# JuliaReinforcementLearning/ReinforcementLearning.jl

Measured on NVIDIA H100. Metric: env-steps/sec at 65536 CartPole envs (full PPO iteration: rollout T=32 + GAE + 4 epochs x 4 minibatches), higher is better.
Workload: dtype f32

## Files before the change

### reinforcementlearning.jl_b200/csrc/nn_tc.cu

```cuda
#include "nn.cuh"
#include "perm.cuh"
#include "policy.cuh"
#include "tc_fwd.cuh"
#include "tc_split.h"
#include "wgmma.cuh"

namespace {

using tcfwd::G_F;
using tcfwd::GW_S;
using tcfwd::WIMG_BYTES;
using tcfwd::split2;
using tcfwd::wimg_off;
constexpr int TM = tcfwd::TM;
constexpr int H = tcfwd::H;
constexpr float kScaleW = tcfwd::kScale;

constexpr int NT7 = 512;
constexpr int kMaxStage = 10;
constexpr int GF_T = 128;
constexpr int GS_T = 16 * GF_T;
constexpr int FIMG = 8 * GS_T;
constexpr float kScaleH = 64.0f, kScaleX = 64.0f;
constexpr int kNo = 2;

struct SmemBwd {
    static_assert(FIMG % 128 == 0 && WIMG_BYTES % 128 == 0 && (2 * GS_T) % 16 == 0, "operand images must stay 128-byte aligned");
    alignas(128) uint8_t FP_full[FIMG];
    alignas(128) uint8_t FP_lo[FIMG];
    alignas(128) uint8_t AH[2][2][FIMG];
    alignas(128) uint8_t FQ_full[FIMG];
    alignas(128) uint8_t FQ_lo[FIMG];
    alignas(128) uint8_t B1[WIMG_BYTES];
    alignas(128) uint8_t XT[2][2 * GS_T];
    alignas(16) float D[TM * H];
    uint64_t H1pos[2][TM];
    float W1[kInMax * H];
    float b1[H], b2[H];
    float W3[H * kNo];
    float b3[kNo];
    float Zp[4 * kNo * TM];
    float Red[32];
    double RedD[16];
    float step_scale;
    alignas(8) uint64_t bar1[2];
    alignas(8) uint64_t bar3;
    alignas(8) uint64_t bar4;
    float AccW2[64 * 65 + 64];
    float AccD4[64 * 9];
};
__device__ __forceinline__ int d_off(int s, int col) { return s * H + ((((col >> 2) ^ (s & 15))) << 2) + (col & 3); }
__device__ __forceinline__ void d_ld16(const float* D, int s, int f0, float (&v)[16]) {
#pragma unroll
    for (int u = 0; u < 4; ++u) {
        const float4 q4 = *reinterpret_cast<const float4*>(D + d_off(s, f0 + 4 * u));
        v[4 * u] = q4.x; v[4 * u + 1] = q4.y; v[4 * u + 2] = q4.z; v[4 * u + 3] = q4.w;
    }
}
template <int TB>
__device__ __forceinline__ void gemm_ts3(float (&d)[32], const uint8_t* a_hi, const uint8_t* a_lo, int h, uint64_t dB, uint32_t b_step) {
    const uint64_t dA = wg::make_desc(wg::smem_u32(a_hi) + 8 * h * GF_T, GS_T, GF_T), dAl = wg::make_desc(wg::smem_u32(a_lo) + 8 * h * GF_T, GS_T, GF_T);
    wg::fence();
#pragma unroll
    for (int k = 0; k < 4; ++k) {
        const uint32_t aa = k * 2 * GS_T, bb = k * b_step;
        wg::mma_m64n64k16<0, TB>(d, wg::desc_add(dA, aa), wg::desc_add(dB, bb), k ? 1u : 0u);
        wg::mma_m64n64k16<0, TB>(d, wg::desc_add(dA, aa), wg::desc_add(dB, 8 * GW_S + bb), 1u);
        wg::mma_m64n64k16<0, TB>(d, wg::desc_add(dAl, aa), wg::desc_add(dB, bb), 1u);
    }
    wg::commit();
    wg::wait_all();
}
__device__ __forceinline__ uint32_t fimg_off(int f, int s) { return (uint32_t)((f >> 3) * GS_T + (s >> 3) * GF_T + (s & 7) * 16 + (f & 7) * 2); }
__device__ __forceinline__ void store16_feat(uint8_t* img, int f0, int s, const uint32_t (&v)[8]) {
    uint8_t* p = img + fimg_off(f0, s);
    *reinterpret_cast<uint4*>(p) = make_uint4(v[0], v[1], v[2], v[3]);
    *reinterpret_cast<uint4*>(p + GS_T) = make_uint4(v[4], v[5], v[6], v[7]);
}
using b200perm::perm_index;
using b200perm::perm_index_bits;

__device__ __forceinline__ float lane_transpose_reduce32(float (&v)[32], int lane) {
#pragma unroll
    for (int st = 0; st < 5; ++st) {
        const int half = 16 >> st, off = 16 >> st;
        const bool upper = (lane & off) != 0;
#pragma unroll
        for (int n = 0; n < half; ++n) {
            float send = upper ? v[n] : v[n + half];
            float keep = upper ? v[n + half] : v[n];
            v[n] = keep + __shfl_xor_sync(0xffffffffu, send, off);
        }
    }
    return v[0];
}

__device__ __forceinline__ void worker_sync() { asm volatile("bar.sync 1, 512;" ::: "memory"); }
__device__ __forceinline__ void group_sync(int q) { asm volatile("bar.sync %0, 128;" ::"r"(5 + q) : "memory"); }
__device__ __forceinline__ void ready_arrive(int id) { asm volatile("bar.arrive %0, 384;" ::"r"(id) : "memory"); }
__device__ __forceinline__ void ready_wait(int id) { asm volatile("bar.sync %0, 384;" ::"r"(id) : "memory"); }
#ifdef B200RL_K7_TIMING
__device__ unsigned long long g_k7_phase[40];
__device__ int g_k7_watch = 0;
#define K7_T(i) do { if (tid == (g_k7_watch & 0xFFFF) && (int)blockIdx.x == (g_k7_watch >> 16)) { long long now_ = clock64(); g_k7_phase[i] += (unsigned long long)(now_ - tprev_); tprev_ = now_; } } while (0)
#else
#define K7_T(i) do { } while (0)
#endif
constexpr int NT7_ALL = NT7 + 128;
constexpr int kRegsMma = 64, kRegsWorker = 104;
static_assert(128 * kRegsMma + NT7 * kRegsWorker <= NT7_ALL * 96, "setmaxnreg split must fit the CTA's register allocation");
constexpr int kBarRdyA = 2, kBarRdyB = 9;
constexpr int kBarMma = 4;
__device__ __forceinline__ void mma_sync() { asm volatile("bar.sync %0, 128;" ::"n"(kBarMma) : "memory"); }

template <int ACT>
__global__ void __launch_bounds__(NT7_ALL, 1)
ac_loss_grad_tc_kernel(MlpDesc actor, MlpDesc critic, const float* params , AcHyper hp, AcBatch b, float* partial,
                       float* __restrict__ loss_partial, int64_t np_total, float scale_base ,
                       OptStep st ,
                       int n_actor ) {
    extern __shared__ __align__(1024) unsigned char smem_raw[];
    SmemBwd& sm = *reinterpret_cast<SmemBwd*>(smem_raw);
    const int role = (int)blockIdx.x < n_actor ? 0 : 1;
    const int cta = role ? (int)blockIdx.x - n_actor : (int)blockIdx.x;
    const int nctas = role ? (int)gridDim.x - n_actor : n_actor;
    const int nrows = max(n_actor, (int)gridDim.x - n_actor);
    const float scale_p = scale_base * (role ? 4.0f : 64.0f);
    const MlpDesc d = role ? critic : actor;
    const int act = ACT >= 0 ? ACT : d.act;
    const bool relu = act == B200RL_ACT_RELU;
    const int64_t poff = role ? actor.nparams() : 0;
    const float* __restrict__ p = params + poff;
    const int tid = threadIdx.x, warp = tid >> 5, lane = tid & 31;
    const int q = warp & 3, c = (warp >> 2) & 3;
    const int s = 32 * q + lane;
    const int half = q >> 1;
    {
        const float* b1 = p + (int64_t)H * d.in;
        const float* W2 = b1 + H;
        const float* b2 = W2 + (int64_t)H * H;
        const float s1 = relu ? kScaleH : 1.0f;
        for (int k = tid; k < kInMax * H; k += NT7_ALL) sm.W1[k] = (k / H) < d.in ? p[k] * s1 : 0.f;
        for (int k = tid; k < H; k += NT7_ALL) { sm.b1[k] = b1[k] * s1; sm.b2[k] = b2[k]; }
        for (int k = tid; k < H * kNo; k += NT7_ALL) {
            int j = k / kNo, o = k % kNo;
            sm.W3[k] = o < d.nout ? p[head_w<false>(d, o, j)] : 0.f;
        }
        if (tid < kNo) sm.b3[tid] = tid < d.nout ? p[head_b<false>(d, tid)] : 0.f;
        tcfwd::fill_w2_image<NT7_ALL>(sm.B1, W2);
    }
    if (tid == 32) {
        wg::mbar_init(&sm.bar1[0], 128); wg::mbar_init(&sm.bar1[1], 128); wg::mbar_init(&sm.bar3, 128); wg::mbar_init(&sm.bar4, 128);
    }
    wg::fence_proxy_async();
    __syncthreads();
    const float inv_s1 = 1.0f / (kScaleH * kScaleW), inv_s3 = 1.0f / (scale_p * kScaleH), inv_sp = 1.0f / scale_p, inv_s4 = 1.0f / (scale_p * kScaleX);
    const int64_t ntiles = (b.B + TM - 1) / TM;

    if (warp >= NT7 / 32) {
        asm volatile("setmaxnreg.dec.sync.aligned.u32 %0;" ::"n"(kRegsMma));
        const int t = tid - NT7, row0 = 16 * (t >> 5) + ((t & 31) >> 2), col0 = 2 * (t & 3);
        const uint64_t dB1k = wg::make_desc(wg::smem_u32(sm.B1), G_F, GW_S);
        const uint64_t dB1t = wg::make_desc(wg::smem_u32(sm.B1), GW_S, G_F);
        float dacc[32];
        auto store_d = [&](int h) {
#pragma unroll
            for (int j = 0; j < 8; ++j)
#pragma unroll
                for (int hh = 0; hh < 2; ++hh)
                    *reinterpret_cast<float2*>(sm.D + d_off(64 * h + row0 + 8 * hh, 8 * j + col0)) = make_float2(dacc[4 * j + 2 * hh], dacc[4 * j + 2 * hh + 1]);
        };
        auto gemm1 = [&](int h, int buf) { gemm_ts3<0>(dacc, sm.AH[buf][0], sm.AH[buf][1], h, dB1k, 2 * G_F); };
        auto gemm2 = [&](int h) { gemm_ts3<1>(dacc, sm.FP_full, sm.FP_lo, h, dB1t, 2 * GW_S); };
        auto store_dp1 = [&](int h, int pbuf) {
#pragma unroll
            for (int hh = 0; hh < 2; ++hh) {
                const int ss = 64 * h + row0 + 8 * hh;
                const uint64_t pos = relu ? sm.H1pos[pbuf][ss] >> col0 : 0u;
#pragma unroll
                for (int j = 0; j < 8; ++j) {
                    const uint32_t off = fimg_off(8 * j + col0, ss);
                    float v0 = dacc[4 * j + 2 * hh] * (1.0f / kScaleW), v1 = dacc[4 * j + 2 * hh + 1] * (1.0f / kScaleW);
                    if (relu) {
                        v0 = ((pos >> (8 * j)) & 1u) ? v0 : 0.f;
                        v1 = ((pos >> (8 * j + 1)) & 1u) ? v1 : 0.f;
                    } else {
                        const float inv_h = 1.0f / kScaleH;
                        const float2 hf = __half22float2(*reinterpret_cast<const __half2*>(sm.AH[pbuf][0] + off));
                        const float2 lf = __half22float2(*reinterpret_cast<const __half2*>(sm.AH[pbuf][1] + off));
                        v0 *= dact_f(act, (hf.x + lf.x) * inv_h);
                        v1 *= dact_f(act, (hf.y + lf.y) * inv_h);
                    }
                    uint32_t hi, lo;
                    split2(v0, v1, hi, lo);
                    *reinterpret_cast<uint32_t*>(sm.FQ_full + off) = hi;
                    *reinterpret_cast<uint32_t*>(sm.FQ_lo + off) = lo;
                }
            }
        };
        auto gemm3 = [&](int buf) {
            const uint64_t dPh = wg::make_desc(wg::smem_u32(sm.FP_full), GF_T, GS_T), dPl = wg::make_desc(wg::smem_u32(sm.FP_lo), GF_T, GS_T);
            const uint64_t dHh = wg::make_desc(wg::smem_u32(sm.AH[buf][0]), GF_T, GS_T), dHl = wg::make_desc(wg::smem_u32(sm.AH[buf][1]), GF_T, GS_T);
            wg::fence();
#pragma unroll
            for (int k = 0; k < 8; ++k) {
                const uint32_t a = k * 2 * GF_T;
                wg::mma_m64n64k16<1, 1>(dacc, wg::desc_add(dPh, a), wg::desc_add(dHh, a), k ? 1u : 0u);
                wg::mma_m64n64k16<1, 1>(dacc, wg::desc_add(dPl, a), wg::desc_add(dHh, a), 1u);
                wg::mma_m64n64k16<1, 1>(dacc, wg::desc_add(dPh, a), wg::desc_add(dHl, a), 1u);
            }
            wg::commit();
            wg::wait_all();
#pragma unroll
            for (int j = 0; j < 8; ++j)
#pragma unroll
                for (int hh = 0; hh < 2; ++hh)
#pragma unroll
                    for (int e = 0; e < 2; ++e) sm.AccW2[(row0 + 8 * hh) * 65 + 8 * j + col0 + e] += dacc[4 * j + 2 * hh + e];
            const uint64_t dX = wg::make_desc(wg::smem_u32(sm.XT[buf]), GF_T, GS_T);
            float d8[4] = {0.f, 0.f, 0.f, 0.f};
            wg::fence();
#pragma unroll
            for (int k = 0; k < 8; ++k) {
                const uint32_t a = k * 2 * GF_T;
                wg::mma_m64n8k16<1, 1>(d8, wg::desc_add(dPh, a), wg::desc_add(dX, a), k ? 1u : 0u);
                wg::mma_m64n8k16<1, 1>(d8, wg::desc_add(dPl, a), wg::desc_add(dX, a), 1u);
            }
            wg::commit();
            wg::wait_all();
            if (col0 == 4) {
                sm.AccW2[64 * 65 + row0] += d8[0];
                sm.AccW2[64 * 65 + row0 + 8] += d8[2];
            }
        };
        auto gemm4 = [&](int buf) {
            const uint64_t dQh = wg::make_desc(wg::smem_u32(sm.FQ_full), GF_T, GS_T), dQl = wg::make_desc(wg::smem_u32(sm.FQ_lo), GF_T, GS_T);
            const uint64_t dX = wg::make_desc(wg::smem_u32(sm.XT[buf]), GF_T, GS_T);
            float d4[4] = {0.f, 0.f, 0.f, 0.f};
            wg::fence();
#pragma unroll
            for (int k = 0; k < 8; ++k) {
                const uint32_t a = k * 2 * GF_T;
                wg::mma_m64n8k16<1, 1>(d4, wg::desc_add(dQh, a), wg::desc_add(dX, a), k ? 1u : 0u);
                wg::mma_m64n8k16<1, 1>(d4, wg::desc_add(dQh, a), wg::desc_add(dX, GS_T + a), 1u);
                wg::mma_m64n8k16<1, 1>(d4, wg::desc_add(dQl, a), wg::desc_add(dX, a), 1u);
            }
            wg::commit();
            wg::wait_all();
#pragma unroll
            for (int hh = 0; hh < 2; ++hh)
#pragma unroll
                for (int e = 0; e < 2; ++e)
                    if (col0 + e < 5) sm.AccD4[(row0 + 8 * hh) * 9 + col0 + e] += d4[2 * hh + e];
        };
        if (cta < ntiles) {
            for (int h = 0; h < 2; ++h) {
                ready_wait(kBarRdyB + h);
                gemm1(h, 0); store_d(h);
                wg::mbar_arrive(&sm.bar1[h]);
            }
        }
        int buf = 0;
        for (int64_t tile = cta; tile < ntiles; tile += nctas, buf ^= 1) {
            const bool has_next = tile + nctas < ntiles;
            for (int h = 0; h < 2; ++h) {
                ready_wait(kBarRdyA + h);
                gemm2(h); store_dp1(h, buf);
                if (has_next) {
                    ready_wait(kBarRdyB + h);
                    gemm1(h, buf ^ 1); store_d(h);
                    wg::mbar_arrive(&sm.bar1[h]);
                }
            }
            wg::fence_proxy_async();
            gemm3(buf);
            wg::mbar_arrive(&sm.bar3);
            mma_sync();
            gemm4(buf);
            wg::mbar_arrive(&sm.bar4);
        }
    } else {
    asm volatile("setmaxnreg.inc.sync.aligned.u32 %0;" ::"n"(kRegsWorker));
    float g3[2][16];
    float gb3a0 = 0.f, gb3a1 = 0.f;
#pragma unroll
    for (int k = 0; k < 16; ++k) { g3[0][k] = 0.f; g3[1][k] = 0.f; }
    float l0 = 0.f, l1 = 0.f;
    float mean = 0.f, inv_std = 1.f;
    if (hp.normalize_adv && b.norm2) { mean = b.norm2[0]; inv_std = b.norm2[1]; }
    uint32_t ph1 = 0, ph3 = 0, ph4 = 0;
    bool gemm4_pending = false;
    int xbuf = 0;
    int pbuf = 0;
#ifdef B200RL_K7_TIMING
    long long tprev_ = clock64();
#endif
    const int pbits = b200perm::perm_bits(b.perm_n);
    const uint32_t pkey = ac_perm_key(b);
    auto index_of = [&](int64_t t) -> int32_t {
        const int64_t j = t * TM + s;
        if (t >= ntiles || j >= b.B) return -1;
        return b.idx ? b.idx[j] : (int32_t)perm_index_bits((uint32_t)(b.perm_offset + j), b.perm_n, pkey, pbits);
    };
    auto request = [&](int32_t g, float (&x)[kInMax], float (&a)[4]) {
#pragma unroll
        for (int k = 0; k < kInMax; ++k) { x[k] = 0.f; a[k] = 0.f; }
        if (g < 0) return;
        if (b.rec) {
            const float4 v0 = b.rec[2 * (int64_t)g], v1 = b.rec[2 * (int64_t)g + 1];
            x[0] = v0.x; x[1] = v0.y; x[2] = v0.z; x[3] = v0.w;
            a[0] = v1.x; a[1] = v1.y; a[2] = v1.z; a[3] = v1.w;
        } else {
#pragma unroll
            for (int i = 0; i < kInMax; ++i)
                if (i < b.ns) x[i] = b.states[(int64_t)b.ns * g + i];
            a[0] = reinterpret_cast<const float*>(b.actions)[g];
            a[1] = b.logp_old ? b.logp_old[g] : 0.f;
            a[2] = b.adv[g];
            a[3] = b.ret[g];
        }
    };
    float pfx[kInMax] = {0.f, 0.f, 0.f, 0.f}, pfa[4] = {0.f, 0.f, 0.f, 0.f};
    float aux[4] = {0.f, 0.f, 0.f, 0.f};
    int32_t gi_next = -1;
    bool gemm3_pending = false;
    float* const out = partial + (int64_t)cta * np_total + poff;
    float* const gW1 = out;
    float* const gb1 = out + (int64_t)H * d.in;
    float* const gW2 = gb1 + H;
    float* const gb2 = gW2 + (int64_t)H * H;
    for (int k = tid; k < 64 * 65 + 64; k += NT7) sm.AccW2[k] = 0.f;
    for (int k = tid; k < 64 * 9; k += NT7) sm.AccD4[k] = 0.f;
    float xo[kInMax];
    auto publish = [&](int64_t t) {
#pragma unroll
        for (int i = 0; i < kInMax; ++i) xo[i] = pfx[i];
        aux[0] = pfa[0];
        aux[1] = role == 0 ? pfa[1] : 0.f;
        aux[2] = role == 0 ? (hp.normalize_adv ? (pfa[2] - mean) * inv_std : pfa[2]) : 0.f;
        aux[3] = role == 0 ? 0.f : pfa[3];
        if (c == 0) {
            uint32_t h01, l01, h23, l23;
            split2(xo[0] * kScaleX, xo[1] * kScaleX, h01, l01);
            split2(xo[2] * kScaleX, xo[3] * kScaleX, h23, l23);
            uint8_t* xt = sm.XT[xbuf] + fimg_off(0, s);
            *reinterpret_cast<uint4*>(xt) = make_uint4(h01, h23, 0x3C00u, 0u);
            *reinterpret_cast<uint4*>(xt + GS_T) = make_uint4(l01, l23, 0u, 0u);
        }
        K7_T(16);
        xbuf ^= 1;
        request(gi_next, pfx, pfa);
        gi_next = index_of(t + 2 * nctas);
        K7_T(17);
    };
    auto layer1 = [&]() {
        uint32_t pos = 0;
        uint32_t hi8[8], lo8[8];
#pragma unroll
        for (int ch = 0; ch < 4; ++ch) {
            const int f0 = 16 * c + 4 * ch;
            float4 bb = *reinterpret_cast<const float4*>(sm.b1 + f0);
            float h[4] = {bb.x, bb.y, bb.z, bb.w};
#pragma unroll
            for (int k = 0; k < kInMax; ++k) {
                float4 w = *reinterpret_cast<const float4*>(sm.W1 + k * H + f0);
                h[0] = fmaf(w.x, xo[k], h[0]); h[1] = fmaf(w.y, xo[k], h[1]); h[2] = fmaf(w.z, xo[k], h[2]); h[3] = fmaf(w.w, xo[k], h[3]);
            }
            if (relu) {
#pragma unroll
                for (int e = 0; e < 4; ++e) { pos |= (h[e] > 0.f ? 1u : 0u) << (4 * ch + e); h[e] = fmaxf(h[e], 0.f); }
            } else {
#pragma unroll
                for (int e = 0; e < 4; ++e) h[e] = act_f(act, h[e]) * kScaleH;
            }
            split2(h[0], h[1], hi8[2 * ch], lo8[2 * ch]);
            split2(h[2], h[3], hi8[2 * ch + 1], lo8[2 * ch + 1]);
        }
        if (relu) reinterpret_cast<uint16_t*>(&sm.H1pos[pbuf][s])[c] = (uint16_t)pos;
        store16_feat(sm.AH[pbuf][0], 16 * c, s, hi8);
        store16_feat(sm.AH[pbuf][1], 16 * c, s, lo8);
        pbuf ^= 1;
    };
    if (cta < ntiles) {
        request(index_of(cta), pfx, pfa);
        gi_next = index_of(cta + nctas);
        publish(cta);
        layer1();
        wg::fence_proxy_async();
        ready_arrive(kBarRdyB + half);
    }
#ifdef B200RL_K7_TIMING
    tprev_ = clock64();
#endif
    for (int64_t tile = cta; tile < ntiles; tile += nctas) {
        const bool has_next = tile + nctas < ntiles;
        wg::mbar_wait(&sm.bar1[half], ph1);
        ph1 ^= 1u;
        K7_T(0);
        float h2[16];
        {
            float v[16];
            d_ld16(sm.D, s, 16 * c, v);
            float zp[kNo] = {0.f, 0.f};
#pragma unroll
            for (int k = 0; k < 16; ++k) {
                const int f = 16 * c + k;
                h2[k] = act_f(act, fmaf(v[k], inv_s1, sm.b2[f]));
                float2 w = *reinterpret_cast<const float2*>(sm.W3 + f * kNo);
                zp[0] = fmaf(w.x, h2[k], zp[0]); zp[1] = fmaf(w.y, h2[k], zp[1]);
            }
#pragma unroll
            for (int o = 0; o < kNo; ++o) sm.Zp[(c * kNo + o) * TM + s] = zp[o];
        }
        K7_T(1);
        group_sync(q);
        K7_T(2);
        {
            float z[kNo];
#pragma unroll
            for (int o = 0; o < kNo; ++o)
                z[o] = sm.b3[o] + ((sm.Zp[o * TM + s] + sm.Zp[(kNo + o) * TM + s]) + (sm.Zp[(2 * kNo + o) * TM + s] + sm.Zp[(3 * kNo + o) * TM + s]));
            const bool valid = (tile * TM + s) < b.B;
            const policy::LossOut<kNo> lo_ = policy::sample_loss(actor.heads2, actor.nout, role, hp, b.inv_B, z, aux[0], aux[1], aux[2], aux[3]);
            float dz[kNo];
#pragma unroll
            for (int o = 0; o < kNo; ++o) dz[o] = valid ? lo_.dz[o] : 0.f;
            if (c == 0 && valid) { l0 += lo_.l0; l1 += lo_.l1; gb3a0 += dz[0]; gb3a1 += dz[1]; }
            const float dzs0 = dz[0] * scale_p, dzs1 = dz[1] * scale_p;
            float dp[16];
#pragma unroll
            for (int k = 0; k < 16; ++k) {
                const int f = 16 * c + k;
                float2 w = *reinterpret_cast<const float2*>(sm.W3 + f * kNo);
                const float dh = fmaf(w.x, dzs0, w.y * dzs1);
                dp[k] = relu ? (h2[k] > 0.f ? dh : 0.f) : dh * (1.f - h2[k] * h2[k]);
                g3[0][k] = fmaf(dz[0], h2[k], g3[0][k]);
                g3[1][k] = fmaf(dz[1], h2[k], g3[1][k]);
            }
            uint32_t hi8[8], lo8[8];
#pragma unroll
            for (int m = 0; m < 8; ++m) split2(dp[2 * m], dp[2 * m + 1], hi8[m], lo8[m]);
            K7_T(3);
            if (gemm3_pending) {
                wg::mbar_wait(&sm.bar3, ph3);
                ph3 ^= 1u;
                gemm3_pending = false;
            }
            K7_T(4);
            store16_feat(sm.FP_full, 16 * c, s, hi8);
            store16_feat(sm.FP_lo, 16 * c, s, lo8);
        }
        K7_T(5);
        wg::fence_proxy_async();
        if (gemm4_pending) {
            wg::mbar_wait(&sm.bar4, ph4);
            ph4 ^= 1u;
        }
        K7_T(6);
        ready_arrive(kBarRdyA + half);
        gemm3_pending = true;
        gemm4_pending = true;
        K7_T(7);
        if (has_next) {
            publish(tile + nctas);
            layer1();
            wg::fence_proxy_async();
            K7_T(8);
            ready_arrive(kBarRdyB + half);
            K7_T(9);
        }
#ifdef B200RL_K7_TIMING
        if (tid == (g_k7_watch & 0xFFFF) && (int)blockIdx.x == (g_k7_watch >> 16)) g_k7_phase[15] += 1;
#endif
    }
    if (gemm3_pending) wg::mbar_wait(&sm.bar3, ph3);
    if (gemm4_pending) wg::mbar_wait(&sm.bar4, ph4);
    worker_sync();
    for (int k = tid; k < H * H; k += NT7) gW2[k] = sm.AccW2[(k & 63) * 65 + (k >> 6)] * inv_s3;
    if (tid < H) {
        gb2[tid] = sm.AccW2[64 * 65 + tid] * inv_sp;
        gb1[tid] = sm.AccD4[tid * 9 + 4] * inv_sp;
        for (int i = 0; i < d.in; ++i) gW1[tid + H * i] = sm.AccD4[tid * 9 + i] * inv_s4;
    }
    if (cta >= (int)gridDim.x - nctas) {
        const int64_t ooff = role ? 0 : actor.nparams(), on = role ? actor.nparams() : critic.nparams();
        float* orow = partial + (int64_t)cta * np_total + ooff;
        for (int64_t kk = tid; kk < on; kk += NT7) orow[kk] = 0.f;
    }
    float* red = reinterpret_cast<float*>(sm.FP_full);
    static_assert(offsetof(SmemBwd, XT) - offsetof(SmemBwd, FP_full) >= (2 * TM * 65 + 2 * 8 * 64) * 4, "drain scratch");
    {
        constexpr int RS = 65;
        float* seg = red + 2 * TM * RS;
#pragma unroll
        for (int k = 0; k < 16; ++k) {
            red[0 * TM * RS + s * RS + 16 * c + k] = g3[0][k];
            red[1 * TM * RS + s * RS + 16 * c + k] = g3[1][k];
        }
        worker_sync();
        {
            const int col = tid & 63, g = tid >> 6;
#pragma unroll
            for (int m = 0; m < 2; ++m) {
                float a = 0.f;
#pragma unroll
                for (int ss = 0; ss < 16; ++ss) a += red[m * TM * RS + (16 * g + ss) * RS + col];
                seg[(m * 8 + g) * 64 + col] = a;
            }
        }
        worker_sync();
        if (tid < 2 * H) {
            const int m = tid >> 6, col = tid & 63;
            float a = 0.f;
#pragma unroll
            for (int g = 0; g < 8; ++g) a += seg[(m * 8 + g) * 64 + col];
            if (m < d.nout) out[head_w<false>(d, m, col)] = a;
        }
        worker_sync();
    }
    if (c == 0) { red[s] = gb3a0; red[TM + s] = gb3a1; }
    worker_sync();
    if (warp < d.nout) {
        float a = (red[warp * TM + lane] + red[warp * TM + 32 + lane]) + (red[warp * TM + 64 + lane] + red[warp * TM + 96 + lane]);
#pragma unroll
        for (int o = 16; o > 0; o >>= 1) a += __shfl_xor_sync(0xffffffffu, a, o);
        if (lane == 0) out[head_b<false>(d, warp)] = a;
    }
    float t0 = l0, t1 = l1;
#pragma unroll
    for (int o = 16; o > 0; o >>= 1) { t0 += __shfl_xor_sync(0xffffffffu, t0, o); t1 += __shfl_xor_sync(0xffffffffu, t1, o); }
    worker_sync();
    if (lane == 0) { sm.Red[warp] = t0; sm.Red[16 + warp] = t1; }
    worker_sync();
    if (tid == 0) {
        float a0 = 0.f, a1 = 0.f;
        for (int k = 0; k < 16; ++k) { a0 += sm.Red[k]; a1 += sm.Red[16 + k]; }
        float* lp = loss_partial + (int64_t)blockIdx.x * 4;
        lp[0] = role ? 0.f : a0; lp[1] = role ? 0.f : a1; lp[2] = role ? a0 : 0.f; lp[3] = 0.f;
    }
    if (blockIdx.x == 0)
        for (int k = tid; k < 4 * (2 * nrows - (int)gridDim.x); k += NT7) loss_partial[4 * (int64_t)gridDim.x + k] = 0.f;
    if (st.params) {
        const unsigned int G = gridDim.x;
        K7_T(24);
        worker_sync();
        K7_T(25);
        if (tid == 0) optim::grid_barrier(st.counters, G);
        worker_sync();
        K7_T(26);
        const int per = (int)((np_total + G - 1) / G);
        const int64_t k = (int64_t)blockIdx.x * per + tid;
        const bool mine = tid < per && k < np_total;
        const unsigned int seq = st.tab.nranks > 1 ? *st.seq_ptr + 1u : 0u;
        float* stage = reinterpret_cast<float*>(sm.FP_full);
        const int nstage = per * nrows;
        const int64_t k0 = (int64_t)blockIdx.x * per;
        {
            float t[kMaxStage];
#pragma unroll
            for (int j = 0; j < kMaxStage; ++j) {
                const int e = tid + j * NT7;
                const int row = e / per, col = e - row * per;
                t[j] = (e < nstage && k0 + col < np_total) ? __ldcg(partial + (int64_t)row * np_total + k0 + col) : 0.f;
            }
#pragma unroll
            for (int j = 0; j < kMaxStage; ++j) {
                const int e = tid + j * NT7;
                if (e < nstage) stage[e] = t[j];
            }
        }
        float* lstage = stage + nstage;
        if (blockIdx.x == 0) {
            float t[2];
#pragma unroll
            for (int j = 0; j < 2; ++j) t[j] = tid + j * NT7 < 4 * (int)G ? __ldcg(loss_partial + tid + j * NT7) : 0.f;
#pragma unroll
            for (int j = 0; j < 2; ++j) if (tid + j * NT7 < 4 * (int)G) lstage[tid + j * NT7] = t[j];
        }
        float m_k = 0.f, v_k = 0.f, p_k = 0.f;
        if (mine) { m_k = st.m[k]; v_k = st.v[k]; p_k = st.params[k]; }
        worker_sync();
        K7_T(27);
        float gk = 0.f;
        if (mine) {
            for (int c0 = 0; c0 < nrows; c0 += 8) {
                float t[8];
#pragma unroll
                for (int j = 0; j < 8; ++j) t[j] = c0 + j < nrows ? stage[(c0 + j) * per + tid] : 0.f;
#pragma unroll
                for (int j = 0; j < 8; ++j) if (c0 + j < nrows) gk += t[j];
            }
        }
        float lsum = 0.f;
        const bool loss_thread = blockIdx.x == 0 && tid < 4;
        if (loss_thread) {
            for (unsigned int c0 = 0; c0 < G; c0 += 8) {
                float t[8];
#pragma unroll
                for (int j = 0; j < 8; ++j) t[j] = c0 + j < G ? lstage[(c0 + j) * 4 + tid] : 0.f;
#pragma unroll
                for (int j = 0; j < 8; ++j) if (c0 + j < G) lsum += t[j];
            }
        }
        if (st.tab.nranks > 1) {
            const unsigned slot = seq & 1u;
            if (mine) p2p_push(st.tab, 0, slot, (size_t)k, __float_as_uint(gk), seq);
            if (loss_thread) p2p_push(st.tab, 0, slot, (size_t)np_total + tid, __float_as_uint(lsum), seq);
            if (mine) gk = p2p_sum_ranks(st.tab, 0, slot, (size_t)k, gk, seq);
            if (loss_thread) lsum = p2p_sum_ranks(st.tab, 0, slot, (size_t)np_total + tid, lsum, seq);
        }
        if (loss_thread) optim::publish_loss(st, tid, lsum);
        double sq = (double)gk * (double)gk;
#pragma unroll
        for (int o = 16; o > 0; o >>= 1) sq += __shfl_xor_sync(0xffffffffu, sq, o);
        if (lane == 0) sm.RedD[warp] = sq;
        worker_sync();
        K7_T(28);
        if (warp == 0) {
            if (lane == 0) {
                double t = 0.0;
                for (int w = 0; w < NT7 / 32; ++w) t += sm.RedD[w];
                st.cta_sumsq[blockIdx.x] = t;
                optim::grid_barrier(st.counters + 1, G);
            }
            __syncwarp();
            K7_T(29);
            double part[8];
#pragma unroll
            for (int j = 0; j < 8; ++j) part[j] = (unsigned)(lane + 32 * j) < G ? __ldcg(st.cta_sumsq + lane + 32 * j) : 0.0;
            double tot = 0.0;
#pragma unroll
            for (int j = 0; j < 8; ++j) tot += part[j];
#pragma unroll
// ... 80 lines not shown
```

### reinforcementlearning.jl_b200/csrc/wgmma.cuh

```cuda
#pragma once
#include <cuda_fp16.h>
#include <cuda_runtime.h>

#include <cstdint>

namespace wg {

__device__ __forceinline__ uint32_t smem_u32(const void* p) { return (uint32_t)__cvta_generic_to_shared(p); }

__device__ __forceinline__ uint64_t make_desc(uint32_t smem_addr, uint32_t lbo_bytes, uint32_t sbo_bytes) {
    uint64_t d = 0;
    d |= (uint64_t)((smem_addr >> 4) & 0x3FFF);
    d |= (uint64_t)((lbo_bytes >> 4) & 0x3FFF) << 16;
    d |= (uint64_t)((sbo_bytes >> 4) & 0x3FFF) << 32;
    return d;
}
__device__ __forceinline__ uint64_t desc_add(uint64_t d, uint32_t bytes) { return d + (uint64_t)(bytes >> 4); }

__device__ __forceinline__ void fence() { asm volatile("wgmma.fence.sync.aligned;" ::: "memory"); }
__device__ __forceinline__ void commit() { asm volatile("wgmma.commit_group.sync.aligned;" ::: "memory"); }
__device__ __forceinline__ void wait_all() { asm volatile("wgmma.wait_group.sync.aligned 0;" ::: "memory"); }
__device__ __forceinline__ void fence_proxy_async() { asm volatile("fence.proxy.async.shared::cta;" ::: "memory"); }

template <int TA, int TB>
__device__ __forceinline__ void mma_m64n8k16(float (&d)[4], uint64_t a_desc, uint64_t b_desc, uint32_t accumulate) {
    asm volatile(
        "{\n\t"
        ".reg .pred p;\n\t"
        "setp.ne.b32 p, %6, 0;\n\t"
        "wgmma.mma_async.sync.aligned.m64n8k16.f32.f16.f16 "
        "{%0, %1, %2, %3}, "
        "%4, %5, p, 1, 1, %7, %8;\n"
        "}\n"
        : "+f"(d[0]), "+f"(d[1]), "+f"(d[2]), "+f"(d[3])
        : "l"(a_desc), "l"(b_desc), "r"(accumulate), "n"(TA), "n"(TB)
        : "memory");
}
template <int TA, int TB>
__device__ __forceinline__ void mma_m64n64k16(float (&d)[32], uint64_t a_desc, uint64_t b_desc, uint32_t accumulate) {
    asm volatile(
        "{\n\t"
        ".reg .pred p;\n\t"
        "setp.ne.b32 p, %34, 0;\n\t"
        "wgmma.mma_async.sync.aligned.m64n64k16.f32.f16.f16 "
        "{%0, %1, %2, %3, %4, %5, %6, %7, %8, %9, %10, %11, %12, %13, %14, %15, "
        "%16, %17, %18, %19, %20, %21, %22, %23, %24, %25, %26, %27, %28, %29, %30, %31}, "
        "%32, %33, p, 1, 1, %35, %36;\n"
        "}\n"
        : "+f"(d[0]), "+f"(d[1]), "+f"(d[2]), "+f"(d[3]), "+f"(d[4]), "+f"(d[5]), "+f"(d[6]), "+f"(d[7]), "+f"(d[8]), "+f"(d[9]),
          "+f"(d[10]), "+f"(d[11]), "+f"(d[12]), "+f"(d[13]), "+f"(d[14]), "+f"(d[15]), "+f"(d[16]), "+f"(d[17]), "+f"(d[18]), "+f"(d[19]),
          "+f"(d[20]), "+f"(d[21]), "+f"(d[22]), "+f"(d[23]), "+f"(d[24]), "+f"(d[25]), "+f"(d[26]), "+f"(d[27]), "+f"(d[28]), "+f"(d[29]),
          "+f"(d[30]), "+f"(d[31])
        : "l"(a_desc), "l"(b_desc), "r"(accumulate), "n"(TA), "n"(TB)
        : "memory");
}


__device__ __forceinline__ void mbar_init(uint64_t* mbar, uint32_t count) {
    asm volatile("mbarrier.init.shared::cta.b64 [%0], %1;" ::"r"(smem_u32(mbar)), "r"(count) : "memory");
    asm volatile("fence.mbarrier_init.release.cluster;" ::: "memory");
}
__device__ __forceinline__ void mbar_arrive(uint64_t* mbar) {
    asm volatile("{\n\t.reg .b64 st;\n\tmbarrier.arrive.shared::cta.b64 st, [%0];\n\t}" ::"r"(smem_u32(mbar)) : "memory");
}
__device__ __forceinline__ bool mbar_try_wait(uint64_t* mbar, uint32_t parity) {
    uint32_t ok;
    asm volatile(
        "{\n\t"
        ".reg .pred p;\n\t"
        "mbarrier.try_wait.parity.shared::cta.b64 p, [%1], %2;\n\t"
        "selp.u32 %0, 1, 0, p;\n\t"
        "}\n"
        : "=r"(ok)
        : "r"(smem_u32(mbar)), "r"(parity)
        : "memory");
    return ok != 0;
}
__device__ __forceinline__ void mbar_wait(uint64_t* mbar, uint32_t parity) {
    for (uint32_t spin = 0; !mbar_try_wait(mbar, parity); ++spin)
        if (spin > (1u << 24)) __trap();
}

}
```

Baseline: 321.4 million.

## Specialize K7 worker warps: one gathers minibatch rows via cp.async, one computes loss

In the backward loss/grad kernel, each worker quadrant's warps now take roles. The gatherer warp prefetches the next tile's samples with cp.async into shared memory and publishes X and aux values. The lead warp alone evaluates the per-sample policy loss and shares dz with the other warps through shared memory. This is meant to remove redundant loss computation and register-held global loads from every warp, at the cost of an extra group_sync per tile and more shared memory. It also adds an offline SASS instruction-budget script.

Measured after the change: 325.7 million (median of 6 runs). +1.3%, better.

```diff
diff --git a/k7_sass_budget.py b/k7_sass_budget.py
--- /dev/null
+++ b/k7_sass_budget.py
@@ -0,0 +1,157 @@
+import argparse
+import collections
+import json
+import os
+import re
+import shutil
+import subprocess
+import sys
+import tempfile
+
+ROOT = os.path.dirname(os.path.abspath(__file__))
+PKG = os.path.join(ROOT, "reinforcementlearning.jl_b200")
+sys.path.insert(0, PKG)
+import build as B
+
+ACTS = {"ILi0E": "relu", "ILi1E": "tanh", "ILin1E": "runtime"}
+CLASSES = [
+    ("fp32", {"FFMA", "FADD", "FMUL", "FMNMX", "FSEL", "FSETP", "FSET", "FCHK", "FRND", "FSWZADD"}),
+    ("conv", {"F2FP", "HADD2", "HMUL2", "HFMA2", "F2F", "F2I", "I2F", "I2FP", "F2IP"}),
+    ("mufu", {"MUFU"}),
+    ("lds_sts", {"LDS", "STS", "LDSM", "STSM"}),
+    ("ldg_stg", {"LDG", "STG", "LD", "ST", "RED", "ATOM", "ATOMG", "ATOMS", "LDGSTS"}),
+    ("local", {"LDL", "STL"}),
+    ("barrier", {"BAR", "SYNCS", "MEMBAR", "FENCE", "WARPSYNC", "BSSY", "BSYNC", "NANOSLEEP", "DEPBAR", "WARPGROUP", "ERRBAR", "CCTL"}),
+    ("branch", {"BRA", "EXIT", "RET", "CALL", "BRX", "JMP"}),
+    ("hgmma", {"HGMMA"}),
+    ("nop", {"NOP"}),
+]
+INS = re.compile(r"/\*([0-9a-f]{4,})\*/\s+(@!?U?P[T0-9]\s+)?([A-Z0-9_]+)(\.[A-Z0-9_.]+)?\s*([^;]*);")
+ROLES = "const bool lead = c == 0, gatherer = c == 1;"
+PATHS = (("c0", "true", "false", 1), ("c1", "false", "true", 1), ("other", "false", "false", 2))
+
+
+def klass(op):
+    for name, ops in CLASSES:
+        if op in ops:
+            return name
+    return "int"
+
+
+def compile_sass(csrc, tmp, tag, patch=None):
+    src_dir = os.path.join(tmp, tag)
+    shutil.copytree(csrc, src_dir)
+    path = os.path.join(src_dir, "nn_tc.cu")
+    if patch:
+        text = open(path).read()
+        open(path, "w").write(text.replace(*patch))
+    cubin = os.path.join(src_dir, "nn_tc.cubin")
+    host_cxx = "/usr/bin/g++" if os.path.exists("/usr/bin/g++") else "g++"
+    inc = ["-I", os.path.join(os.path.dirname(os.path.dirname(os.path.abspath(csrc))), "include"), "-I", os.path.abspath(csrc)]
+    subprocess.check_call([B._nvcc(), "-ccbin", host_cxx] + B.ARCH + B.COMMON + inc + ["-cubin", path, "-o", cubin])
+    nvcc = B._nvcc()
+    cuobjdump = os.path.join(os.path.dirname(nvcc), "cuobjdump") if os.path.isabs(nvcc) else "cuobjdump"
+    return subprocess.check_output([cuobjdump, "-sass", cubin], text=True)
+
+
+def functions(sass):
+    out, cur = {}, None
+    for line in sass.splitlines():
+        if "Function :" in line:
+            name = line.split("Function :")[1].strip()
+            cur = next((v for k, v in ACTS.items() if k in name), None) if "ac_loss_grad_tc_kernel" in name else None
+            if cur:
+                out[cur] = []
+            continue
+        m = INS.search(line) if cur else None
+        if m:
+            out[cur].append((int(m.group(1), 16), bool(m.group(2)), m.group(3), m.group(4) or "", m.group(5)))
+    return out
+
+
+def natural_loops(ins):
+    at = {x[0]: i for i, x in enumerate(ins)}
+    succ = [[] for _ in ins]
+    for i, (a, pred, op, _m, opnds) in enumerate(ins):
+        tgt = re.search(r"0x([0-9a-f]+)", opnds) if op == "BRA" else None
+        if tgt and int(tgt.group(1), 16) in at:
+            succ[i].append(at[int(tgt.group(1), 16)])
+        if not (op in ("BRA", "EXIT", "RET", "BRX", "JMP") and not pred) and i + 1 < len(ins):
+            succ[i].append(i + 1)
+    preds = [[] for _ in ins]
+    for i, ss in enumerate(succ):
+        for j in ss:
+            preds[j].append(i)
+    loops = []
+    for i, ss in enumerate(succ):
+        for h in ss:
+            if h <= i:
+                body, stack = {h, i}, [i]
+                while stack:
+                    n = stack.pop()
+                    for p in preds[n]:
+                        if p not in body:
+                            body.add(p)
+                            stack.append(p)
+                loops.append(body)
+    return loops
+
+
+def count(ins, body):
+    sel = [ins[i] for i in sorted(body)]
+    return {"instructions": len(sel), "by_class": dict(collections.Counter(klass(x[2]) for x in sel).most_common()),
+            "top_opcodes": dict(collections.Counter(x[2] for x in sel).most_common(14))}
+
+
+def budget(ins):
+    waits = {i: re.search(r"\+0x([0-9a-f]+)\]", x[4]) for i, x in enumerate(ins) if x[2] == "SYNCS" and "TRYWAIT" in x[3]}
+    offs = {i: int(m.group(1), 16) for i, m in waits.items() if m}
+    bar1 = min(offs.values())
+    bar1_waits = {i for i, o in offs.items() if o == bar1}
+    hgmma = {i for i, x in enumerate(ins) if x[2] == "HGMMA"}
+    loops = [lp for lp in natural_loops(ins) if 0 not in lp]
+    worker = max((lp for lp in loops if lp & bar1_waits and not lp & hgmma), key=len)
+    mma = max((lp for lp in loops if lp & hgmma), key=len)
+    return {"worker_loop": count(ins, worker), "mma_loop": count(ins, mma)}
+
+
+def main():
+    ap = argparse.ArgumentParser()
+    ap.add_argument("--src", default=B.CSRC, help="csrc directory to count (default: this checkout's)")
+    ap.add_argument("--json", action="store_true")
+    a = ap.parse_args()
+    csrc = os.path.abspath(a.src)
+    with tempfile.TemporaryDirectory() as tmp:
+        res = {k: budget(v) for k, v in functions(compile_sass(csrc, tmp, "as_is")).items()}
+        has_roles = ROLES in open(os.path.join(csrc, "nn_tc.cu")).read()
+        paths = {}
+        if has_roles:
+            for tag, lead, gath, _n in PATHS:
+                for act, ins in functions(compile_sass(csrc, tmp, tag, (ROLES, f"const bool lead = {lead}, gatherer = {gath};"))).items():
+                    paths.setdefault(act, {})[tag] = budget(ins)["worker_loop"]
+    for act, r in res.items():
+        w = r["worker_loop"]
+        if has_roles:
+            pa = r["worker_paths"] = paths[act]
+            cls = sorted(set().union(*(pa[t]["by_class"] for t, *_ in PATHS)))
+            r["quadrant_issue_per_tile"] = {"instructions": sum(n * pa[t]["instructions"] for t, _l, _g, n in PATHS),
+                                            "by_class": {k: sum(n * pa[t]["by_class"].get(k, 0) for t, _l, _g, n in PATHS) for k in cls}}
+        else:
+            r["quadrant_issue_per_tile"] = {"instructions": 4 * w["instructions"], "by_class": {k: 4 * v for k, v in sorted(w["by_class"].items())}}
+    if a.json:
+        print(json.dumps(res))
+        return
+    print(f"K7 SASS budget of {csrc} (static counts per tile)")
+    for act in ("relu", "tanh", "runtime"):
+        r = res[act]
+        print(f"== {act}")
+        rows = [("worker loop", r["worker_loop"]), ("MMA loop", r["mma_loop"])]
+        if "worker_paths" in r:
+            rows += [(f"  {t} path", r["worker_paths"][t]) for t, *_ in PATHS]
+        rows.append(("quadrant: 4 worker warps", r["quadrant_issue_per_tile"]))
+        for name, x in rows:
+            print(f"  {name:26s} {x['instructions']:6d}   " + "  ".join(f"{k} {v}" for k, v in x["by_class"].items()))
+
+
+if __name__ == "__main__":
+    main()
diff --git a/reinforcementlearning.jl_b200/csrc/nn_tc.cu b/reinforcementlearning.jl_b200/csrc/nn_tc.cu
--- a/reinforcementlearning.jl_b200/csrc/nn_tc.cu
+++ b/reinforcementlearning.jl_b200/csrc/nn_tc.cu
@@ -40,6 +40,10 @@
     float W3[H * kNo];
     float b3[kNo];
     float Zp[4 * kNo * TM];
+    float Xn[kInMax * TM];
+    float DZ[kNo * TM];
+    float4 Rec[2 * TM];
+    float4 Aux[2][TM];
     float Red[32];
     double RedD[16];
     float step_scale;
@@ -49,6 +53,7 @@
     float AccW2[64 * 65 + 64];
     float AccD4[64 * 9];
 };
+static_assert(sizeof(SmemBwd) + 128 <= 227 * 1024, "K7's shared memory must fit one CTA per SM");
 __device__ __forceinline__ int d_off(int s, int col) { return s * H + ((((col >> 2) ^ (s & 15))) << 2) + (col & 3); }
 __device__ __forceinline__ void d_ld16(const float* D, int s, int f0, float (&v)[16]) {
 #pragma unroll
@@ -77,6 +82,13 @@
     *reinterpret_cast<uint4*>(p) = make_uint4(v[0], v[1], v[2], v[3]);
     *reinterpret_cast<uint4*>(p + GS_T) = make_uint4(v[4], v[5], v[6], v[7]);
 }
+__device__ __forceinline__ void cp_async16(void* dst, const void* src) {
+    asm volatile("cp.async.cg.shared.global [%0], [%1], 16;" ::"r"(wg::smem_u32(dst)), "l"(src) : "memory");
+}
+__device__ __forceinline__ void cp_async4(void* dst, const void* src) {
+    asm volatile("cp.async.ca.shared.global [%0], [%1], 4;" ::"r"(wg::smem_u32(dst)), "l"(src) : "memory");
+}
+__device__ __forceinline__ void cp_async_wait_all() { asm volatile("cp.async.wait_all;" ::: "memory"); }
 using b200perm::perm_index;
 using b200perm::perm_index_bits;
 
@@ -292,6 +304,8 @@
     bool gemm4_pending = false;
     int xbuf = 0;
     int pbuf = 0;
+    const bool lead = c == 0, gatherer = c == 1;
+    int abuf = 0;
 #ifdef B200RL_K7_TIMING
     long long tprev_ = clock64();
 #endif
@@ -302,26 +316,27 @@
         if (t >= ntiles || j >= b.B) return -1;
         return b.idx ? b.idx[j] : (int32_t)perm_index_bits((uint32_t)(b.perm_offset + j), b.perm_n, pkey, pbits);
     };
-    auto request = [&](int32_t g, float (&x)[kInMax], float (&a)[4]) {
-#pragma unroll
-        for (int k = 0; k < kInMax; ++k) { x[k] = 0.f; a[k] = 0.f; }
-        if (g < 0) return;
-        if (b.rec) {
-            const float4 v0 = b.rec[2 * (int64_t)g], v1 = b.rec[2 * (int64_t)g + 1];
-            x[0] = v0.x; x[1] = v0.y; x[2] = v0.z; x[3] = v0.w;
-            a[0] = v1.x; a[1] = v1.y; a[2] = v1.z; a[3] = v1.w;
+    float* const rec_s = reinterpret_cast<float*>(sm.Rec + 2 * s);
+    auto request = [&](int32_t g) {
+        if (g < 0) {
+#pragma unroll
+            for (int k = 0; k < 8; ++k) rec_s[k] = 0.f;
+        } else if (b.rec) {
+            cp_async16(rec_s, b.rec + 2 * (int64_t)g);
+            cp_async16(rec_s + 4, b.rec + 2 * (int64_t)g + 1);
         } else {
 #pragma unroll
-            for (int i = 0; i < kInMax; ++i)
-                if (i < b.ns) x[i] = b.states[(int64_t)b.ns * g + i];
-            a[0] = reinterpret_cast<const float*>(b.actions)[g];
-            a[1] = b.logp_old ? b.logp_old[g] : 0.f;
-            a[2] = b.adv[g];
-            a[3] = b.ret[g];
+            for (int i = 0; i < kInMax; ++i) {
+                if (i < b.ns) cp_async4(rec_s + i, b.states + (int64_t)b.ns * g + i);
+                else rec_s[i] = 0.f;
+            }
+            cp_async4(rec_s + 4, reinterpret_cast<const float*>(b.actions) + g);
+            if (b.logp_old) cp_async4(rec_s + 5, b.logp_old + g);
+            else rec_s[5] = 0.f;
+            cp_async4(rec_s + 6, b.adv + g);
+            cp_async4(rec_s + 7, b.ret + g);
         }
     };
-    float pfx[kInMax] = {0.f, 0.f, 0.f, 0.f}, pfa[4] = {0.f, 0.f, 0.f, 0.f};
-    float aux[4] = {0.f, 0.f, 0.f, 0.f};
     int32_t gi_next = -1;
     bool gemm3_pending = false;
     float* const out = partial + (int64_t)cta * np_total + poff;
@@ -331,15 +346,20 @@
     float* const gb2 = gW2 + (int64_t)H * H;
     for (int k = tid; k < 64 * 65 + 64; k += NT7) sm.AccW2[k] = 0.f;
     for (int k = tid; k < 64 * 9; k += NT7) sm.AccD4[k] = 0.f;
+    auto pass_next = [&](int64_t t, int ab) {
+        cp_async_wait_all();
+        const float4 x4 = sm.Rec[2 * s], a4 = sm.Rec[2 * s + 1];
+        sm.Xn[0 * TM + s] = x4.x; sm.Xn[1 * TM + s] = x4.y; sm.Xn[2 * TM + s] = x4.z; sm.Xn[3 * TM + s] = x4.w;
+        sm.Aux[ab][s] = make_float4(a4.x, role == 0 ? a4.y : 0.f, role == 0 ? (hp.normalize_adv ? (a4.z - mean) * inv_std : a4.z) : 0.f,
+                                    role == 0 ? 0.f : a4.w);
+        request(gi_next);
+        gi_next = index_of(t + 2 * nctas);
+    };
     float xo[kInMax];
-    auto publish = [&](int64_t t) {
-#pragma unroll
-        for (int i = 0; i < kInMax; ++i) xo[i] = pfx[i];
-        aux[0] = pfa[0];
-        aux[1] = role == 0 ? pfa[1] : 0.f;
-        aux[2] = role == 0 ? (hp.normalize_adv ? (pfa[2] - mean) * inv_std : pfa[2]) : 0.f;
-        aux[3] = role == 0 ? 0.f : pfa[3];
-        if (c == 0) {
+    auto publish = [&]() {
+#pragma unroll
+        for (int i = 0; i < kInMax; ++i) xo[i] = sm.Xn[i * TM + s];
+        if (gatherer) {
             uint32_t h01, l01, h23, l23;
             split2(xo[0] * kScaleX, xo[1] * kScaleX, h01, l01);
             split2(xo[2] * kScaleX, xo[3] * kScaleX, h23, l23);
@@ -347,11 +367,8 @@
             *reinterpret_cast<uint4*>(xt) = make_uint4(h01, h23, 0x3C00u, 0u);
             *reinterpret_cast<uint4*>(xt + GS_T) = make_uint4(l01, l23, 0u, 0u);
         }
+        xbuf ^= 1;
         K7_T(16);
-        xbuf ^= 1;
-        request(gi_next, pfx, pfa);
-        gi_next = index_of(t + 2 * nctas);
-        K7_T(17);
     };
     auto layer1 = [&]() {
         uint32_t pos = 0;
@@ -382,9 +399,13 @@
         pbuf ^= 1;
     };
     if (cta < ntiles) {
-        request(index_of(cta), pfx, pfa);
-        gi_next = index_of(cta + nctas);
-        publish(cta);
+        if (gatherer) {
+            request(index_of(cta));
+            gi_next = index_of(cta + nctas);
+            pass_next(cta, 0);
+        }
+        group_sync(q);
+        publish();
         layer1();
         wg::fence_proxy_async();
         ready_arrive(kBarRdyB + half);
@@ -416,16 +437,25 @@
         group_sync(q);
         K7_T(2);
         {
-            float z[kNo];
-#pragma unroll
-            for (int o = 0; o < kNo; ++o)
-                z[o] = sm.b3[o] + ((sm.Zp[o * TM + s] + sm.Zp[(kNo + o) * TM + s]) + (sm.Zp[(2 * kNo + o) * TM + s] + sm.Zp[(3 * kNo + o) * TM + s]));
-            const bool valid = (tile * TM + s) < b.B;
-            const policy::LossOut<kNo> lo_ = policy::sample_loss(actor.heads2, actor.nout, role, hp, b.inv_B, z, aux[0], aux[1], aux[2], aux[3]);
             float dz[kNo];
-#pragma unroll
-            for (int o = 0; o < kNo; ++o) dz[o] = valid ? lo_.dz[o] : 0.f;
-            if (c == 0 && valid) { l0 += lo_.l0; l1 += lo_.l1; gb3a0 += dz[0]; gb3a1 += dz[1]; }
+            if (gatherer) pass_next(tile + nctas, abuf ^ 1);
+            if (lead) {
+                float z[kNo];
+#pragma unroll
+                for (int o = 0; o < kNo; ++o)
+                    z[o] = sm.b3[o] + ((sm.Zp[o * TM + s] + sm.Zp[(kNo + o) * TM + s]) + (sm.Zp[(2 * kNo + o) * TM + s] + sm.Zp[(3 * kNo + o) * TM + s]));
+                const bool valid = (tile * TM + s) < b.B;
+                const float4 aux = sm.Aux[abuf][s];
+                const policy::LossOut<kNo> lo_ = policy::sample_loss(actor.heads2, actor.nout, role, hp, b.inv_B, z, aux.x, aux.y, aux.z, aux.w);
+#pragma unroll
+                for (int o = 0; o < kNo; ++o) { dz[o] = valid ? lo_.dz[o] : 0.f; sm.DZ[o * TM + s] = dz[o]; }
+                if (valid) { l0 += lo_.l0; l1 += lo_.l1; gb3a0 += dz[0]; gb3a1 += dz[1]; }
+            }
+            group_sync(q);
+            if (!lead) {
+#pragma unroll
+                for (int o = 0; o < kNo; ++o) dz[o] = sm.DZ[o * TM + s];
+            }
             const float dzs0 = dz[0] * scale_p, dzs1 = dz[1] * scale_p;
             float dp[16];
 #pragma unroll
@@ -462,13 +492,14 @@
         gemm4_pending = true;
         K7_T(7);
         if (has_next) {
-            publish(tile + nctas);
+            publish();
             layer1();
             wg::fence_proxy_async();
             K7_T(8);
             ready_arrive(kBarRdyB + half);
             K7_T(9);
         }
+        abuf ^= 1;
 #ifdef B200RL_K7_TIMING
         if (tid == (g_k7_watch & 0xFFFF) && (int)blockIdx.x == (g_k7_watch >> 16)) g_k7_phase[15] += 1;
 #endif
```

## Merge gemm3/gemm4 with overlapped accumulation and specialize loss by head count

Applied to the files above, without the earlier changes.

Fuses the weight-gradient GEMMs into one routine that issues the W2 and bias MMAs back to back, waiting on only the first group before accumulating into shared memory, so the accumulate overlaps the second MMA group. The AccW2 stride changes from 65 to 72 so accumulation can use float2 read-modify-writes. The worker loss computation is also templated on the number of outputs so the single-head role skips the second-head arithmetic. The padded stride alters bank-conflict behaviour and uses a little more shared memory, and the barrier arrival points move.

Measured after the change: 320.8 million before, 334.3 million after, median of 6. 1.04x the previous value.

```diff
diff --git a/reinforcementlearning.jl_b200/csrc/nn_tc.cu b/reinforcementlearning.jl_b200/csrc/nn_tc.cu
--- a/reinforcementlearning.jl_b200/csrc/nn_tc.cu
+++ b/reinforcementlearning.jl_b200/csrc/nn_tc.cu
@@ -22,6 +22,7 @@
 constexpr int GS_T = 16 * GF_T;
 constexpr int FIMG = 8 * GS_T;
 constexpr float kScaleH = 64.0f, kScaleX = 64.0f;
+constexpr int kAccW2S = 72;
 constexpr int kNo = 2;
 
 struct SmemBwd {
@@ -46,7 +47,7 @@
     alignas(8) uint64_t bar1[2];
     alignas(8) uint64_t bar3;
     alignas(8) uint64_t bar4;
-    float AccW2[64 * 65 + 64];
+    alignas(8) float AccW2[64 * kAccW2S + 64];
     float AccD4[64 * 9];
 };
 __device__ __forceinline__ int d_off(int s, int col) { return s * H + ((((col >> 2) ^ (s & 15))) << 2) + (col & 3); }
@@ -198,9 +199,12 @@
                 }
             }
         };
-        auto gemm3 = [&](int buf) {
+        auto gemm34 = [&](int buf) {
             const uint64_t dPh = wg::make_desc(wg::smem_u32(sm.FP_full), GF_T, GS_T), dPl = wg::make_desc(wg::smem_u32(sm.FP_lo), GF_T, GS_T);
             const uint64_t dHh = wg::make_desc(wg::smem_u32(sm.AH[buf][0]), GF_T, GS_T), dHl = wg::make_desc(wg::smem_u32(sm.AH[buf][1]), GF_T, GS_T);
+            const uint64_t dQh = wg::make_desc(wg::smem_u32(sm.FQ_full), GF_T, GS_T), dQl = wg::make_desc(wg::smem_u32(sm.FQ_lo), GF_T, GS_T);
+            const uint64_t dX = wg::make_desc(wg::smem_u32(sm.XT[buf]), GF_T, GS_T);
+            float d8[4] = {0.f, 0.f, 0.f, 0.f}, d4[4] = {0.f, 0.f, 0.f, 0.f};
             wg::fence();
 #pragma unroll
             for (int k = 0; k < 8; ++k) {
@@ -210,16 +214,6 @@
                 wg::mma_m64n64k16<1, 1>(dacc, wg::desc_add(dPh, a), wg::desc_add(dHl, a), 1u);
             }
             wg::commit();
-            wg::wait_all();
-#pragma unroll
-            for (int j = 0; j < 8; ++j)
-#pragma unroll
-                for (int hh = 0; hh < 2; ++hh)
-#pragma unroll
-                    for (int e = 0; e < 2; ++e) sm.AccW2[(row0 + 8 * hh) * 65 + 8 * j + col0 + e] += dacc[4 * j + 2 * hh + e];
-            const uint64_t dX = wg::make_desc(wg::smem_u32(sm.XT[buf]), GF_T, GS_T);
-            float d8[4] = {0.f, 0.f, 0.f, 0.f};
-            wg::fence();
 #pragma unroll
             for (int k = 0; k < 8; ++k) {
                 const uint32_t a = k * 2 * GF_T;
@@ -227,16 +221,23 @@
                 wg::mma_m64n8k16<1, 1>(d8, wg::desc_add(dPl, a), wg::desc_add(dX, a), 1u);
             }
             wg::commit();
+            wg::wait_groups<1>();
+#pragma unroll
+            for (int j = 0; j < 8; ++j)
+#pragma unroll
+                for (int hh = 0; hh < 2; ++hh) {
+                    float2* a = reinterpret_cast<float2*>(sm.AccW2 + (row0 + 8 * hh) * kAccW2S + 8 * j + col0);
+                    float2 v = *a;
+                    v.x += dacc[4 * j + 2 * hh];
+                    v.y += dacc[4 * j + 2 * hh + 1];
+                    *a = v;
+                }
             wg::wait_all();
             if (col0 == 4) {
-                sm.AccW2[64 * 65 + row0] += d8[0];
-                sm.AccW2[64 * 65 + row0 + 8] += d8[2];
-            }
-        };
-        auto gemm4 = [&](int buf) {
-            const uint64_t dQh = wg::make_desc(wg::smem_u32(sm.FQ_full), GF_T, GS_T), dQl = wg::make_desc(wg::smem_u32(sm.FQ_lo), GF_T, GS_T);
-            const uint64_t dX = wg::make_desc(wg::smem_u32(sm.XT[buf]), GF_T, GS_T);
-            float d4[4] = {0.f, 0.f, 0.f, 0.f};
+                sm.AccW2[64 * kAccW2S + row0] += d8[0];
+                sm.AccW2[64 * kAccW2S + row0 + 8] += d8[2];
+            }
+            wg::mbar_arrive(&sm.bar3);
             wg::fence();
 #pragma unroll
             for (int k = 0; k < 8; ++k) {
@@ -252,6 +253,7 @@
 #pragma unroll
                 for (int e = 0; e < 2; ++e)
                     if (col0 + e < 5) sm.AccD4[(row0 + 8 * hh) * 9 + col0 + e] += d4[2 * hh + e];
+            wg::mbar_arrive(&sm.bar4);
         };
         if (cta < ntiles) {
             for (int h = 0; h < 2; ++h) {
@@ -273,11 +275,8 @@
                 }
             }
             wg::fence_proxy_async();
-            gemm3(buf);
-            wg::mbar_arrive(&sm.bar3);
             mma_sync();
-            gemm4(buf);
-            wg::mbar_arrive(&sm.bar4);
+            gemm34(buf);
         }
     } else {
     asm volatile("setmaxnreg.inc.sync.aligned.u32 %0;" ::"n"(kRegsWorker));
@@ -329,7 +328,7 @@
     float* const gb1 = out + (int64_t)H * d.in;
     float* const gW2 = gb1 + H;
     float* const gb2 = gW2 + (int64_t)H * H;
-    for (int k = tid; k < 64 * 65 + 64; k += NT7) sm.AccW2[k] = 0.f;
+    for (int k = tid; k < 64 * kAccW2S + 64; k += NT7) sm.AccW2[k] = 0.f;
     for (int k = tid; k < 64 * 9; k += NT7) sm.AccD4[k] = 0.f;
     float xo[kInMax];
     auto publish = [&](int64_t t) {
@@ -392,54 +391,73 @@
 #ifdef B200RL_K7_TIMING
     tprev_ = clock64();
 #endif
+    auto tile_loss = [&](auto no, int64_t tile, uint32_t(&hi8)[8], uint32_t(&lo8)[8]) {
+        constexpr int NO = decltype(no)::value;
+        float h2[16];
+        {
+            float v[16];
+            d_ld16(sm.D, s, 16 * c, v);
+            float zp[NO];
+#pragma unroll
+            for (int o = 0; o < NO; ++o) zp[o] = 0.f;
+#pragma unroll
+            for (int k = 0; k < 16; ++k) {
+                const int f = 16 * c + k;
+                h2[k] = act_f(act, fmaf(v[k], inv_s1, sm.b2[f]));
+                if constexpr (NO == 2) {
+                    float2 w = *reinterpret_cast<const float2*>(sm.W3 + f * kNo);
+                    zp[0] = fmaf(w.x, h2[k], zp[0]); zp[1] = fmaf(w.y, h2[k], zp[1]);
+                } else {
+                    zp[0] = fmaf(sm.W3[f * kNo], h2[k], zp[0]);
+                }
+            }
+#pragma unroll
+            for (int o = 0; o < NO; ++o) sm.Zp[(c * kNo + o) * TM + s] = zp[o];
+        }
+        K7_T(1);
+        group_sync(q);
+        K7_T(2);
+        float z[kNo] = {0.f, 0.f};
+#pragma unroll
+        for (int o = 0; o < NO; ++o)
+            z[o] = sm.b3[o] + ((sm.Zp[o * TM + s] + sm.Zp[(kNo + o) * TM + s]) + (sm.Zp[(2 * kNo + o) * TM + s] + sm.Zp[(3 * kNo + o) * TM + s]));
+        const bool valid = (tile * TM + s) < b.B;
+        const policy::LossOut<kNo> lo_ = policy::sample_loss(actor.heads2, actor.nout, NO == 2 ? 0 : 1, hp, b.inv_B, z, aux[0], aux[1], aux[2], aux[3]);
+        float dz[kNo];
+#pragma unroll
+        for (int o = 0; o < kNo; ++o) dz[o] = valid ? lo_.dz[o] : 0.f;
+        if (c == 0 && valid) {
+            l0 += lo_.l0; gb3a0 += dz[0];
+            if constexpr (NO == 2) { l1 += lo_.l1; gb3a1 += dz[1]; }
+        }
+        const float dzs0 = dz[0] * scale_p, dzs1 = dz[1] * scale_p;
+        float dp[16];
+#pragma unroll
+        for (int k = 0; k < 16; ++k) {
+            const int f = 16 * c + k;
+            float dh;
+            if constexpr (NO == 2) {
+                float2 w = *reinterpret_cast<const float2*>(sm.W3 + f * kNo);
+                dh = fmaf(w.x, dzs0, w.y * dzs1);
+            } else {
+                dh = fmaf(sm.W3[f * kNo], dzs0, 0.f);
+            }
+            dp[k] = relu ? (h2[k] > 0.f ? dh : 0.f) : dh * (1.f - h2[k] * h2[k]);
+            g3[0][k] = fmaf(dz[0], h2[k], g3[0][k]);
+            if constexpr (NO == 2) g3[1][k] = fmaf(dz[1], h2[k], g3[1][k]);
+        }
+#pragma unroll
+        for (int m = 0; m < 8; ++m) split2(dp[2 * m], dp[2 * m + 1], hi8[m], lo8[m]);
+    };
     for (int64_t tile = cta; tile < ntiles; tile += nctas) {
         const bool has_next = tile + nctas < ntiles;
         wg::mbar_wait(&sm.bar1[half], ph1);
         ph1 ^= 1u;
         K7_T(0);
-        float h2[16];
         {
-            float v[16];
-            d_ld16(sm.D, s, 16 * c, v);
-            float zp[kNo] = {0.f, 0.f};
-#pragma unroll
-            for (int k = 0; k < 16; ++k) {
-                const int f = 16 * c + k;
-                h2[k] = act_f(act, fmaf(v[k], inv_s1, sm.b2[f]));
-                float2 w = *reinterpret_cast<const float2*>(sm.W3 + f * kNo);
-                zp[0] = fmaf(w.x, h2[k], zp[0]); zp[1] = fmaf(w.y, h2[k], zp[1]);
-            }
-#pragma unroll
-            for (int o = 0; o < kNo; ++o) sm.Zp[(c * kNo + o) * TM + s] = zp[o];
-        }
-        K7_T(1);
-        group_sync(q);
-        K7_T(2);
-        {
-            float z[kNo];
-#pragma unroll
-            for (int o = 0; o < kNo; ++o)
-                z[o] = sm.b3[o] + ((sm.Zp[o * TM + s] + sm.Zp[(kNo + o) * TM + s]) + (sm.Zp[(2 * kNo + o) * TM + s] + sm.Zp[(3 * kNo + o) * TM + s]));
-            const bool valid = (tile * TM + s) < b.B;
-            const policy::LossOut<kNo> lo_ = policy::sample_loss(actor.heads2, actor.nout, role, hp, b.inv_B, z, aux[0], aux[1], aux[2], aux[3]);
-            float dz[kNo];
-#pragma unroll
-            for (int o = 0; o < kNo; ++o) dz[o] = valid ? lo_.dz[o] : 0.f;
-            if (c == 0 && valid) { l0 += lo_.l0; l1 += lo_.l1; gb3a0 += dz[0]; gb3a1 += dz[1]; }
-            const float dzs0 = dz[0] * scale_p, dzs1 = dz[1] * scale_p;
-            float dp[16];
-#pragma unroll
-            for (int k = 0; k < 16; ++k) {
-                const int f = 16 * c + k;
-                float2 w = *reinterpret_cast<const float2*>(sm.W3 + f * kNo);
-                const float dh = fmaf(w.x, dzs0, w.y * dzs1);
-                dp[k] = relu ? (h2[k] > 0.f ? dh : 0.f) : dh * (1.f - h2[k] * h2[k]);
-                g3[0][k] = fmaf(dz[0], h2[k], g3[0][k]);
-                g3[1][k] = fmaf(dz[1], h2[k], g3[1][k]);
-            }
             uint32_t hi8[8], lo8[8];
-#pragma unroll
-            for (int m = 0; m < 8; ++m) split2(dp[2 * m], dp[2 * m + 1], hi8[m], lo8[m]);
+            if (role) tile_loss(std::integral_constant<int, 1>{}, tile, hi8, lo8);
+            else tile_loss(std::integral_constant<int, 2>{}, tile, hi8, lo8);
             K7_T(3);
             if (gemm3_pending) {
                 wg::mbar_wait(&sm.bar3, ph3);
@@ -476,9 +494,9 @@
     if (gemm3_pending) wg::mbar_wait(&sm.bar3, ph3);
     if (gemm4_pending) wg::mbar_wait(&sm.bar4, ph4);
     worker_sync();
-    for (int k = tid; k < H * H; k += NT7) gW2[k] = sm.AccW2[(k & 63) * 65 + (k >> 6)] * inv_s3;
+    for (int k = tid; k < H * H; k += NT7) gW2[k] = sm.AccW2[(k & 63) * kAccW2S + (k >> 6)] * inv_s3;
     if (tid < H) {
-        gb2[tid] = sm.AccW2[64 * 65 + tid] * inv_sp;
+        gb2[tid] = sm.AccW2[64 * kAccW2S + tid] * inv_sp;
         gb1[tid] = sm.AccD4[tid * 9 + 4] * inv_sp;
         for (int i = 0; i < d.in; ++i) gW1[tid + H * i] = sm.AccD4[tid * 9 + i] * inv_s4;
     }
diff --git a/reinforcementlearning.jl_b200/csrc/wgmma.cuh b/reinforcementlearning.jl_b200/csrc/wgmma.cuh
--- a/reinforcementlearning.jl_b200/csrc/wgmma.cuh
+++ b/reinforcementlearning.jl_b200/csrc/wgmma.cuh
@@ -20,6 +20,8 @@
 __device__ __forceinline__ void fence() { asm volatile("wgmma.fence.sync.aligned;" ::: "memory"); }
 __device__ __forceinline__ void commit() { asm volatile("wgmma.commit_group.sync.aligned;" ::: "memory"); }
 __device__ __forceinline__ void wait_all() { asm volatile("wgmma.wait_group.sync.aligned 0;" ::: "memory"); }
+template <int N>
+__device__ __forceinline__ void wait_groups() { asm volatile("wgmma.wait_group.sync.aligned %0;" ::"n"(N) : "memory"); }
 __device__ __forceinline__ void fence_proxy_async() { asm volatile("fence.proxy.async.shared::cta;" ::: "memory"); }
 
 template <int TA, int TB>
```
